# Anonymousijcai2024ttnet/scale_imagenet

Measured on AMD Instinct MI355X. Metric: images/sec ImageNet 224x224, TT-small, MI355X; top-1 exact-match, higher is better.
Workload: dtype u16/u32/u64 packed bits (gate path); f32 as prescaled fp16x2 split operands on the 16-bit MFMA (stem, lin1, lin2); 1 GPU; TT_general_imagenet_v2_small forward, batch=256 224x224 per GPU, bit-packed HIP LUT kernels (BASELINE.json configs[1]); batch_per_gpu=256, global_batch=256, batches_in_flight=2, input=float32 NCHW, normalised (the reference's contract), parallelism=batch shard x1

## Files before the change

scale_imagenet_amd/csrc/head.hip:

```cpp

#include <algorithm>
#include <cmath>
#include <type_traits>

#include "ttnet_common.h"

namespace ttnet {

namespace {

typedef float f32x16 __attribute__((ext_vector_type(16)));

typedef _Float16 f16x8 __attribute__((ext_vector_type(8)));
constexpr int NP = SPLIT_PLANES;

#ifndef TT_LIN1_SKIP
#define TT_LIN1_SKIP 0
#endif
constexpr int kLin1Skip = TT_LIN1_SKIP;

#ifndef TT_LIN1_BM
#define TT_LIN1_BM 128
#endif
#ifndef TT_LIN1_WGS
#define TT_LIN1_WGS 256
#endif
constexpr int G_BM = TT_LIN1_BM, G_BN = 128;
constexpr int G_MT = G_BM / 32, G_NT = G_BN / 32;
constexpr int G_KS = 1;
constexpr int G_CHUNK = 1024;
constexpr int G_STAGE = (G_MT + G_NT) * G_KS * NP * G_CHUNK;
#ifndef TT_LIN1_STAGES
#define TT_LIN1_STAGES 4
#endif
constexpr int G_STAGES = TT_LIN1_STAGES;
#ifndef TT_LIN1_WAVES
#define TT_LIN1_WAVES (TT_LIN1_BM / 32)
#endif
constexpr int G_WAVES = TT_LIN1_WAVES;
constexpr int G_WN = G_WAVES / G_MT, NPW = G_NT / G_WN;
static_assert(G_WAVES % G_MT == 0 && G_NT % G_WN == 0, "waves tile the workgroup's output");
constexpr int G_CHUNKS = (G_MT + G_NT) * G_KS * NP;
#ifndef TT_LIN1_LOADERS
#define TT_LIN1_LOADERS 0
#endif
constexpr int G_LOADERS = TT_LIN1_LOADERS;
constexpr int G_THREADS = 64 * (G_WAVES + G_LOADERS);
constexpr int G_LW = G_LOADERS ? G_LOADERS : G_WAVES;
constexpr int G_LOADS = (G_CHUNKS + G_LW - 1) / G_LW;
constexpr int G_LDS = G_STAGES * G_STAGE + G_CHUNK;

#ifdef TT_LIN1_STAMP
__device__ unsigned long long g_lin1_stamps[512][2];
#endif
template <int AUX_A, int AUX_B>
__global__ __launch_bounds__(G_THREADS) void gemm_f16x2_kernel(const uint8_t *__restrict__ Af, const uint8_t *__restrict__ Bf,
                                                         float *__restrict__ part, int M, int N, int KS, int ks_per,
                                                         int n_tiles, int m_tiles, int splits) {
  extern __shared__ __align__(16) uint8_t lds[];
  const int lane = threadIdx.x & 63, wave = __builtin_amdgcn_readfirstlane(threadIdx.x >> 6);
  const bool loader = G_LOADERS ? wave >= G_WAVES : true, consumer = wave < G_WAVES;
  const int lw = G_LOADERS ? (loader ? wave - G_WAVES : 0) : wave;
  int ntile, mtile, slice;
  {
    const int b = blockIdx.x, groups = m_tiles * splits;
    const int lanes8 = groups < 8 ? groups : 8;
    const int round = b / (lanes8 * n_tiles), rem = b % (lanes8 * n_tiles);
    int grp = round * lanes8 + rem % lanes8;
    ntile = rem / lanes8;
    if (round == groups / lanes8) {
      const int left = groups - round * lanes8;
      grp = round * lanes8 + rem % left;
      ntile = rem / left;
    }
    mtile = grp / splits;
    slice = grp % splits;
  }
  const int mt0 = mtile * G_MT, nt0 = ntile * G_NT;
  const int ks_beg = slice * ks_per, iters = ks_per / G_KS;

  const uint8_t *chunk_src[G_LOADS];
  int chunk_lds[G_LOADS];
#pragma unroll
  for (int jj = 0; jj < G_LOADS; ++jj) {
    const int c = lw + G_LW * jj;
    const bool real = c < G_CHUNKS;
    const bool isA = c < G_MT * G_KS * NP;
    const int cc = real ? (isA ? c : c - G_MT * G_KS * NP) : 0;
    const int pl = cc % NP, kk = (cc / NP) % G_KS, tl = cc / (NP * G_KS);
    chunk_src[jj] = (isA || !real ? Af : Bf) +
                    ((((size_t)((isA || !real ? mt0 : nt0) + tl) * KS + ks_beg + kk) * NP + pl) * 64 + lane) * 16;
    chunk_lds[jj] = real ? c * G_CHUNK : -1;
  }
  auto issue = [&](int it, int buf) {
    static_for<0, G_LOADS>([&](auto jc) {
      constexpr int jj = decltype(jc)::value;
      constexpr bool allA = G_LW * jj + G_LW - 1 < G_MT * G_KS * NP, allB = G_LW * jj >= G_MT * G_KS * NP;
      if constexpr (kLin1Skip & 3) {
        const bool isA = lw + G_LW * jj < G_MT * G_KS * NP;
        if (((kLin1Skip & 1) && isA) || ((kLin1Skip & 2) && !isA)) return;
      }
      const auto src = (const __attribute__((address_space(1))) void *)(chunk_src[jj] + (size_t)it * (G_KS * NP * G_CHUNK));
      const auto dst = (__attribute__((address_space(3))) void *)(lds + (chunk_lds[jj] >= 0 ? buf * G_STAGE + chunk_lds[jj] : G_STAGES * G_STAGE));
      if constexpr (allA) __builtin_amdgcn_global_load_lds(src, dst, 16, 0, AUX_A);
      else if constexpr (allB) __builtin_amdgcn_global_load_lds(src, dst, 16, 0, AUX_B);
      else __builtin_amdgcn_global_load_lds(src, dst, 16, 0, 0);
    });
  };

  constexpr int MPW = 1;
  const int wm = wave % G_MT, wn = wave / G_MT;
  f32x16 acc[MPW][NPW];
#pragma unroll
  for (int i = 0; i < MPW; ++i)
#pragma unroll
    for (int j = 0; j < NPW; ++j)
#pragma unroll
      for (int r = 0; r < 16; ++r) acc[i][j][r] = 0.f;

  static_assert(G_KS == 1 && MPW == 1 && NPW == 4, "the fragment pipeline below is written for one k-step per stage and four N-tiles per wave");
  auto wait_landed = [&](int younger) {
    if (younger >= 5) asm volatile("s_waitcnt vmcnt(%0)" ::"n"(5 * G_LOADS) : "memory");
    else if (younger == 4) asm volatile("s_waitcnt vmcnt(%0)" ::"n"(4 * G_LOADS) : "memory");
    else if (younger == 3) asm volatile("s_waitcnt vmcnt(%0)" ::"n"(3 * G_LOADS) : "memory");
    else if (younger == 2) asm volatile("s_waitcnt vmcnt(%0)" ::"n"(2 * G_LOADS) : "memory");
    else if (younger == 1) asm volatile("s_waitcnt vmcnt(%0)" ::"n"(G_LOADS) : "memory");
    else asm volatile("s_waitcnt vmcnt(0)" ::: "memory");
  };
  static_assert(G_STAGES >= 4 && G_STAGES <= 8 && 5 * G_LOADS < 64, "G_STAGES - 1 stages issued ahead; the barrier of k-step it frees slot (it - 1) % G_STAGES");
#ifdef TT_LIN1_STAMP
  const unsigned long long st_c = __builtin_amdgcn_s_memtime(), st_r = __builtin_amdgcn_s_memrealtime();
#endif
  if (loader) {
    for (int p = 0; p < G_STAGES - 1 && p < iters; ++p) issue(p, p);
    wait_landed(min(G_STAGES - 2, iters - 1));
  }
  __builtin_amdgcn_s_barrier();
  typedef uint32_t u32x4 __attribute__((ext_vector_type(4)));
  u32x4 af[2][NP], bq[NPW][NP];
#define TT_DSRD(dst, addr, off) asm volatile("ds_read_b128 %0, %1 offset:%2" : "=&v"(dst) : "v"(addr), "n"(off))
  const uint32_t lds0 = (uint32_t)(uintptr_t)(__attribute__((address_space(3))) void *)lds + (uint32_t)lane * 16u;
  const uint32_t offA = (uint32_t)(wm * NP) * G_CHUNK, offB = (uint32_t)(G_MT * NP + wn * NPW * NP) * G_CHUNK;
  auto tile = [&](int j, const u32x4 (&a_cur)[NP]) {
    if constexpr (kLin1Skip & 4) {
      acc[0][j][0] += __uint_as_float(a_cur[0][0] ^ bq[j][0][0] ^ bq[j][1][0] ^ a_cur[1][0]);
    } else {
      const f16x8 a0 = __builtin_bit_cast(f16x8, a_cur[0]), a1 = __builtin_bit_cast(f16x8, a_cur[1]);
      const f16x8 b0 = __builtin_bit_cast(f16x8, bq[j][0]), b1 = __builtin_bit_cast(f16x8, bq[j][1]);
      acc[0][j] = __builtin_amdgcn_mfma_f32_32x32x16_f16(a1, b0, acc[0][j], 0, 0, 0);
      acc[0][j] = __builtin_amdgcn_mfma_f32_32x32x16_f16(a0, b1, acc[0][j], 0, 0, 0);
      acc[0][j] = __builtin_amdgcn_mfma_f32_32x32x16_f16(a0, b0, acc[0][j], 0, 0, 0);
    }
    __builtin_amdgcn_sched_barrier(0);
  };
  auto kstep = [&](auto par_c, int it) {
    constexpr int P = decltype(par_c)::value;
    u32x4 (&a_cur)[NP] = af[P];
    u32x4 (&a_nxt)[NP] = af[1 - P];
    const uint32_t sb = lds0 + (uint32_t)(it % G_STAGES) * G_STAGE + offB;
    const uint32_t sn = lds0 + (uint32_t)((it + 1) % G_STAGES) * G_STAGE;
    const uint32_t snb = sn + offB, sna = sn + offA;
    TT_DSRD(bq[2][0], sb, 4 * G_CHUNK);
    TT_DSRD(bq[2][1], sb, 5 * G_CHUNK);
    asm volatile("s_waitcnt lgkmcnt(4)" : "+v"(bq[0][0]), "+v"(bq[0][1]), "+v"(a_cur[0]), "+v"(a_cur[1]));
    tile(0, a_cur);
    TT_DSRD(bq[3][0], sb, 6 * G_CHUNK);
    TT_DSRD(bq[3][1], sb, 7 * G_CHUNK);
    asm volatile("s_waitcnt lgkmcnt(4)" : "+v"(bq[1][0]), "+v"(bq[1][1]));
    tile(1, a_cur);
    TT_DSRD(bq[0][0], snb, 0);
    TT_DSRD(bq[0][1], snb, G_CHUNK);
    TT_DSRD(a_nxt[0], sna, 0);
    TT_DSRD(a_nxt[1], sna, G_CHUNK);
    asm volatile("s_waitcnt lgkmcnt(6)" : "+v"(bq[2][0]), "+v"(bq[2][1]));
    tile(2, a_cur);
    TT_DSRD(bq[1][0], snb, 2 * G_CHUNK);
    TT_DSRD(bq[1][1], snb, 3 * G_CHUNK);
    asm volatile("s_waitcnt lgkmcnt(6)" : "+v"(bq[3][0]), "+v"(bq[3][1]));
    tile(3, a_cur);
  };
  if (consumer) {
    const uint32_t s0 = lds0;
    TT_DSRD(bq[0][0], s0 + offB, 0);
    TT_DSRD(bq[0][1], s0 + offB, G_CHUNK);
    TT_DSRD(af[0][0], s0 + offA, 0);
    TT_DSRD(af[0][1], s0 + offA, G_CHUNK);
    TT_DSRD(bq[1][0], s0 + offB, 2 * G_CHUNK);
    TT_DSRD(bq[1][1], s0 + offB, 3 * G_CHUNK);
  }
  auto step = [&](auto par_c, int it) {
    if (loader) wait_landed(max(0, min(it + G_STAGES - 2, iters - 1) - (it + 1)));
    __builtin_amdgcn_s_barrier();
    if (loader && it + G_STAGES - 1 < iters) issue(it + G_STAGES - 1, (it + G_STAGES - 1) % G_STAGES);
    if (consumer) kstep(par_c, it);
  };
#pragma unroll 1
  for (int it = 0; it < iters; it += 2) {
    step(std::integral_constant<int, 0>{}, it);
    if (it + 1 < iters) step(std::integral_constant<int, 1>{}, it + 1);
  }
  if (consumer)
    asm volatile("s_waitcnt lgkmcnt(0)" : "+v"(bq[0][0]), "+v"(bq[0][1]), "+v"(bq[1][0]), "+v"(bq[1][1]), "+v"(af[0][0]), "+v"(af[0][1]),
                 "+v"(af[1][0]), "+v"(af[1][1]));
#undef TT_DSRD
#ifdef TT_LIN1_STAMP
  if (threadIdx.x == 0 && blockIdx.x < 512) {
    g_lin1_stamps[blockIdx.x][0] = __builtin_amdgcn_s_memtime() - st_c;
    g_lin1_stamps[blockIdx.x][1] = 10ull * (__builtin_amdgcn_s_memrealtime() - st_r);
  }
#endif
  if (!consumer) return;
  float4 *dst = (float4 *)part + (size_t)slice * (m_tiles * G_MT) * (n_tiles * G_NT) * 256;
#pragma unroll
  for (int i = 0; i < MPW; ++i)
#pragma unroll
    for (int j = 0; j < NPW; ++j) {
      float4 *tile = dst + ((size_t)(mt0 + wm + i) * (n_tiles * G_NT) + nt0 + wn * NPW + j) * 256 + lane;
#pragma unroll
      for (int g = 0; g < 4; ++g) {
        if ((kLin1Skip & 8) && g) continue;
        tile[g * 64] = make_float4(acc[i][j][4 * g], acc[i][j][4 * g + 1], acc[i][j][4 * g + 2], acc[i][j][4 * g + 3]);
      }
    }
}

__global__ void split_to_frag_kernel(const float *__restrict__ src, uint16_t *__restrict__ dst, int R, int K, int tiles,
                                     float prescale, int ld, int kvalid) {
  const size_t i = (size_t)blockIdx.x * blockDim.x + threadIdx.x;
  const int KS = K / 16;
  if (i >= (size_t)tiles * KS * 64 * 8) return;
  const int j = i % 8, ln = (i / 8) % 64;
  const size_t tk = i / 512;
  const int ks = tk % KS, tl = tk / KS;
  const int row = tl * 32 + (ln & 31), k = ks * 16 + 8 * (ln >> 5) + j;
  const float v = row < R && k < kvalid ? src[(size_t)row * ld + k] * prescale : 0.f;
  uint16_t h1, h2;
  split_f16x2(v, h1, h2);
  const size_t base = ((size_t)tl * KS + ks) * NP;
  dst[((base + 0) * 64 + ln) * 8 + j] = h1;
  dst[((base + 1) * 64 + ln) * 8 + j] = h2;
}

__global__ void frag_to_ref_kernel(const uint16_t *__restrict__ af, float *__restrict__ out, int n, int G, int PP) {
  const size_t t = (size_t)blockIdx.x * blockDim.x + threadIdx.x;
  const size_t per = (size_t)G * PP * 16;
  if (t >= (size_t)n * per) return;
  const int kk = t % 16, pp = (t / 16) % PP, g = (t / (16 * (size_t)PP)) % G;
  const int img = t / per;
  out[(size_t)img * per + ((size_t)(16 * g + kk)) * PP + pp] = load_feature(af, img, G * PP, g * PP + pp, kk);
}

__global__ void head_mid_kernel(const float4 *__restrict__ part, int splits, const float *__restrict__ scale,
                                const float *__restrict__ shift, uint16_t *__restrict__ mid_frag, int M, int N,
                                int polynomial, uint32_t *range_flag, int mt32, int nt32) {
  const size_t i = (size_t)blockIdx.x * blockDim.x + threadIdx.x;
  const size_t per_slice = (size_t)mt32 * nt32 * 256;
  if (i >= per_slice) return;
  const int lane = i & 63, g = (i >> 6) & 3;
  const int nt = (int)((i >> 8) % nt32), mt = (int)((i >> 8) / nt32);
  const int col = nt * 32 + (lane & 31), row0 = mt * 32 + 8 * g + 4 * (lane >> 5);
  if (col >= N || row0 >= M) return;
  double s[4] = {0.0, 0.0, 0.0, 0.0};
#pragma unroll 8
  for (int z = 0; z < splits; ++z) {
    const float4 v = part[(size_t)z * per_slice + i];
    s[0] += (double)v.x; s[1] += (double)v.y; s[2] += (double)v.z; s[3] += (double)v.w;
  }
  const float sc = scale[col], sh = shift[col];
#pragma unroll
  for (int e = 0; e < 4; ++e) {
// ... 32 lines not shown
    if (sl < nk) load(sl, fa[sl], fb[sl]);
  });
  for (int i0 = 0; i0 < nk; i0 += L2_STAGES) {
    static_for<0, L2_STAGES>([&](auto ss) {
      constexpr int sl = decltype(ss)::value;
      if (i0 + sl < nk) {
        const f16x8 a0 = __builtin_bit_cast(f16x8, fa[sl][0]), a1 = __builtin_bit_cast(f16x8, fa[sl][1]);
        const f16x8 b0 = __builtin_bit_cast(f16x8, fb[sl][0]), b1 = __builtin_bit_cast(f16x8, fb[sl][1]);
        acc = __builtin_amdgcn_mfma_f32_32x32x16_f16(a1, b0, acc, 0, 0, 0);
        acc = __builtin_amdgcn_mfma_f32_32x32x16_f16(a0, b1, acc, 0, 0, 0);
        acc = __builtin_amdgcn_mfma_f32_32x32x16_f16(a0, b0, acc, 0, 0, 0);
        if (i0 + sl + L2_STAGES < nk) load(i0 + sl + L2_STAGES, fa[sl], fb[sl]);
      }
    });
  }
#pragma unroll
  for (int r = 0; r < 16; ++r) red[(wave * 16 + r) * 64 + lane] = acc[r];
  __syncthreads();
  for (int e = threadIdx.x; e < 16 * 64; e += 64 * L2_WAVES) {
    double sum = 0.0;
#pragma unroll
    for (int w = 0; w < L2_WAVES; ++w) sum += (double)red[w * (16 * 64) + e];
    const int ln = e & 63, r = e >> 6;
    const int row = mt * 32 + (r & 3) + 8 * (r >> 2) + 4 * (ln >> 5);
    const int col = nt * 32 + (ln & 31);
    if (row < M && col < N) out[(size_t)row * N + col] = (float)(sum * (double)inv + (double)bias[col]);
  }
}

__global__ void permute_lin1_kernel(const float *__restrict__ w1, float *__restrict__ w1p, int O, int G, int PP) {
  const size_t i = (size_t)blockIdx.x * blockDim.x + threadIdx.x;
  const size_t K = (size_t)G * PP * 16;
  if (i >= (size_t)O * K) return;
  const size_t o = i / K, f = i % K;
  const int k = f % 16, pp = (f / 16) % PP, g = f / (16 * (size_t)PP);
  w1p[i] = w1[o * K + ((size_t)(16 * g + k)) * PP + pp];
}

}

int gemm_f16x2_splits(int M, int N, int KS) {
  const int tiles = ((M + G_BM - 1) / G_BM) * ((N + G_BN - 1) / G_BN);
  const int want = std::max(TT_LIN1_WGS / std::max(1, tiles), 8);
  for (int s = std::min(std::min(want, KS / 8), 128); s > 1; --s)
    if (KS % s == 0) return s;
  return 1;
}

size_t gemm_f16x2_part_elems(int M, int N, int KS) {
  const size_t mt = (M + G_BM - 1) / G_BM, nt = (N + G_BN - 1) / G_BN;
  return (size_t)gemm_f16x2_splits(M, N, KS) * mt * G_BM * nt * G_BN;
}

int launch_gemm_f16x2(const void *Af, const void *Bf, float *part, int M, int N, int K, int splits, hipStream_t s) {
  const int KS = K / 16;
  if (K % 16 || KS % splits || (KS / splits) % G_KS) {
    set_error("gemm_f16x2: K=%d not divisible into %d slices of %d k-steps", K, splits, G_KS);
    return TTNET_E_UNSUPPORTED;
  }
  static const int nt = getenv("TTNET_LIN1_NT") ? atoi(getenv("TTNET_LIN1_NT")) : 0;
  const int n_tiles = (N + G_BN - 1) / G_BN, m_tiles = (M + G_BM - 1) / G_BM;
  auto launch = [&](auto kernel) -> int {
    TT_TRY(ensure_dynamic_lds((const void *)kernel, G_LDS));
    hipLaunchKernelGGL(kernel, dim3(n_tiles * m_tiles * splits), dim3(G_THREADS), G_LDS, s, (const uint8_t *)Af, (const uint8_t *)Bf, part, M, N,
                       KS, KS / splits, n_tiles, m_tiles, splits);
    return TTNET_OK;
  };
  if (nt == 11) TT_TRY(launch(gemm_f16x2_kernel<2, 2>));
  else if (nt == 1) TT_TRY(launch(gemm_f16x2_kernel<0, 2>));
  else if (nt == 10) TT_TRY(launch(gemm_f16x2_kernel<2, 0>));
  else TT_TRY(launch(gemm_f16x2_kernel<0, 0>));
  TT_HIP(hipGetLastError());
  return TTNET_OK;
}

size_t frag_elems(int rows, int K) { return (size_t)((rows + 31) / 32) * (K / 16) * NP * 64 * 8; }

float weight_prescale(const float *w, size_t n) {
  float amax = 0.f;
  for (size_t i = 0; i < n; ++i) amax = fmaxf(amax, fabsf(w[i]));
  if (!(amax > 0.f) || !std::isfinite(amax)) return 1.0f;
  int e;
  frexpf(amax, &e);
  int k = 14 - e;
  k = k > 60 ? 60 : (k < -60 ? -60 : k);
  return ldexpf(1.0f, k);
}

int launch_split_to_frag(const float *src, void *dst, int R, int K, int rows_padded, float prescale, hipStream_t s, int ld,
                         int kvalid) {
  if (K % 16) {
    set_error("split_to_frag: K=%d is not a multiple of 16", K);
    return TTNET_E_UNSUPPORTED;
  }
  const int tiles = (rows_padded + 31) / 32;
  const size_t t = (size_t)tiles * (K / 16) * 64 * 8;
  hipLaunchKernelGGL(split_to_frag_kernel, dim3((unsigned)((t + 255) / 256)), dim3(256), 0, s, src, (uint16_t *)dst, R, K, tiles,
                     prescale, ld > 0 ? ld : K, kvalid > 0 ? kvalid : K);
  TT_HIP(hipGetLastError());
  return TTNET_OK;
}

int launch_frag_to_reference_order(const void *af, float *out, int n, int G, int PP, hipStream_t s) {
  const size_t t = (size_t)n * G * PP * 16;
  hipLaunchKernelGGL(frag_to_ref_kernel, dim3((unsigned)((t + 255) / 256)), dim3(256), 0, s, (const uint16_t *)af, out, n, G, PP);
  TT_HIP(hipGetLastError());
  return TTNET_OK;
}

int launch_head_mid(const float *part, int splits, const float *scale, const float *shift, void *mid_frag, int M, int N,
                    int polynomial, uint32_t *range_flag, hipStream_t s) {
  const int mt32 = (M + G_BM - 1) / G_BM * G_MT, nt32 = (N + G_BN - 1) / G_BN * G_NT;
  const size_t t = (size_t)mt32 * nt32 * 256;
  hipLaunchKernelGGL(head_mid_kernel, dim3((unsigned)((t + 255) / 256)), dim3(256), 0, s, (const float4 *)part, splits, scale, shift,
                     (uint16_t *)mid_frag, M, N, polynomial, range_flag, mt32, nt32);
  TT_HIP(hipGetLastError());
  return TTNET_OK;
}

int launch_lin2_f16x2(const void *mid_frag, const void *w2f, const float *bias, float inv, float *out, int M, int N, int K,
                      hipStream_t s) {
  const int KS = (K + 15) / 16;
  hipLaunchKernelGGL(lin2_f16x2_kernel, dim3((N + 31) / 32, (M + 31) / 32), dim3(64 * L2_WAVES), 0, s,
                     (const uint4 *)mid_frag, (const uint4 *)w2f, bias, inv, out, M, N, KS);
// ... 19 lines not shown
```

scale_imagenet_amd/csrc/plan.hip:

```cpp

#include <math.h>
#include <stdarg.h>
#include <stdint.h>
#include <stdio.h>
#include <stdlib.h>
#include <string.h>

#include <algorithm>
#include <array>
#include <map>
#include <mutex>
#include <unordered_map>

#include "ttnet_common.h"

namespace ttnet {

static thread_local char g_err[1024] = "";

void set_error(const char *fmt, ...) {
  va_list ap;
  va_start(ap, fmt);
  vsnprintf(g_err, sizeof(g_err), fmt, ap);
  va_end(ap);
// ... 80 lines not shown
  float *full_gel = nullptr;

  uint16_t *stem_wt = nullptr;
  float *stem_init = nullptr;
  uint32_t *norm_tab = nullptr;
  uint16_t *stem_wt_u8 = nullptr;
  float *stem_init_u8 = nullptr;
  float in_mean[3] = {0.485f, 0.456f, 0.406f}, in_std[3] = {0.229f, 0.224f, 0.225f};
  float *w1p = nullptr;
  uint16_t *w1f = nullptr;
  float *bn_scale = nullptr, *bn_shift = nullptr;
  uint16_t *w2f = nullptr;
  float lin2_inv = 1.f;
  size_t part_elems = 0;
  size_t table_bytes = 0, workspace_bytes = 0;
  bool usage_on = false;
  size_t usage_bytes = 0;
  int usage_scheme_dw = kUsageMerged, usage_scheme_pw = kUsageMerged;

  bool profiling = false;
  struct GraphEntry {
    hipGraph_t graph = nullptr;
    hipGraphExec_t exec = nullptr;
    struct Kernel {
      hipGraphNode_t node = nullptr;
      hipKernelNodeParams p{};
      uint64_t argv[12] = {};
      void *args[12] = {};
    };
    Kernel first, last;
    const void *x = nullptr;
    void *out = nullptr;
  };
  struct Lane {
    struct Block {
      uint16_t *o[4] = {nullptr, nullptr, nullptr, nullptr};
      uint64_t *c3_tmp = nullptr;
      uint32_t *idx = nullptr;
    };
    std::vector<uint64_t *> x_rp;
    std::vector<uint16_t *> x_cp;
    std::vector<Block> blk;
    uint64_t *va_y = nullptr;
    float *last_float = nullptr;
    uint32_t *full_fix = nullptr;
    float *part = nullptr;
    uint16_t *feat = nullptr;
    uint16_t *mid_frag = nullptr;
    uint64_t *u_rows = nullptr, *u_br[4] = {nullptr, nullptr, nullptr, nullptr};
    uint32_t *u_tap = nullptr;
    std::map<int64_t, GraphEntry> graphs;
    std::map<int64_t, int> eager_calls;
    int64_t last_n = 0;
  };
  std::vector<Lane> lanes;
  int last_lane = 0;
  hipStream_t cap_stream = nullptr;
  bool graphs_ok = getenv("TTNET_NO_GRAPH") == nullptr;
  int64_t graph_replays = 0;
  int64_t graph_captures = 0, graph_drops = 0;
  std::string graph_off_reason;
  uint32_t *range_host = nullptr, *range_dev = nullptr;
  std::vector<Timing> timings;
  size_t timing_used = 0;

  std::vector<void *> owned;
};

int ttnet::ensure_dynamic_lds(const void *kernel, size_t bytes) {
  if (bytes <= 64 * 1024) return TTNET_OK;
  static std::mutex mu;
  static std::unordered_map<const void *, size_t> done;
  std::lock_guard<std::mutex> lock(mu);
  auto it = done.find(kernel);
  if (it != done.end() && it->second >= bytes) return TTNET_OK;
  TT_HIP(hipFuncSetAttribute(kernel, hipFuncAttributeMaxDynamicSharedMemorySize, (int)bytes));
  done[kernel] = bytes;
  return TTNET_OK;
}

namespace {

template <typename T>
int dev_alloc(ttnet_plan *pl, T **out, size_t count, bool zero, size_t *account = nullptr) {
  void *ptr = nullptr;
  const size_t bytes = std::max<size_t>(count * sizeof(T), 16);
  hipError_t e = hipMalloc(&ptr, bytes);
  if (e != hipSuccess) {
    set_error("hipMalloc(%zu bytes) failed: %s", bytes, hipGetErrorString(e));
    return TTNET_E_NOMEM;
  }
  if (zero) TT_HIP(hipMemset(ptr, 0, bytes));
  pl->owned.push_back(ptr);
  if (account) *account += bytes;
  *out = (T *)ptr;
  return TTNET_OK;
}

void dev_free(ttnet_plan *pl, void *ptr) {
  if (!ptr) return;
  auto it = std::find(pl->owned.begin(), pl->owned.end(), ptr);
  if (it != pl->owned.end()) pl->owned.erase(it);
  (void)hipFree(ptr);
}

void add_tensor(ttnet_plan *pl, const std::string &key, std::vector<int64_t> shape, int dtype, bool required) {
// ... 582 lines not shown
  }
  {
    FullPwArgs a = pw_args(mh.c3, mh.H, mh.W);
    a.interleaved = 0; a.src[0] = L.x_rp[i];
    a.out_rp = c3_tmp; a.out_float = nullptr;
    static const char *const kC3[4] = {"full.conv3.f4", "full.conv3.f5", "full.conv3.f6", "full.conv3.f7"};
    TT_TIMED(pl, kC3[std::min<size_t>(i, 3)], s, launch_full_pw(a, s));
    TT_TIMED(pl, "full.maj3", s,
             launch_rp_majority(c3_tmp, o64[2], n, mh.C, mh.H, mh.W, mh.Ho, mh.off34, mh.off34, s));
    TT_TIMED(pl, "full.maj4", s,
             launch_rp_majority(L.x_rp[i], o64[3], n, mh.C, mh.H, mh.W, mh.Ho, mh.off34, mh.off34, s));
  }
  {
    FullPwArgs a = pw_args(mh.cf, mh.Ho, mh.Wo);
    a.interleaved = 1;
    for (int k = 0; k < 4; ++k) a.src[k] = o64[k];
    if (mh.last) {
      a.out_rp = nullptr; a.out_float = L.last_float;
      TT_TIMED(pl, "full.convf_last", s, launch_full_pw(a, s));
      TT_TIMED(pl, "full.pool", s, launch_full_pool_split(L.last_float, L.feat, n, mh.cf.g.out_planes, mh.Ho, mh.Wo, pl->range_dev, s));
    } else {
      a.out_rp = L.x_rp[i + 1]; a.out_float = nullptr;
      static const char *const kCf[4] = {"full.convf.f4", "full.convf.f5", "full.convf.f6", "full.convf.f7"};
      TT_TIMED(pl, kCf[std::min<size_t>(i, 3)], s, launch_full_pw(a, s));
    }
  }
  return TTNET_OK;
}

int prepare_head(ttnet_plan *pl, hipStream_t s) {
  const Tensor &t1 = pl->tensors[pl->head + ".lin1.weight"], &t2 = pl->tensors[pl->head + ".lin2.weight"];
  std::vector<double> sc, sh;
  TT_TRY(fold_bn(pl, pl->head + ".BN2", sc, sh));
  std::vector<float> w;
  TT_TRY(fetch(t1, w));
  const float ws1 = weight_prescale(w.data(), w.size());
  for (double &v : sc) v /= (double)ws1 * ACT_PRESCALE;
  TT_TRY(upload_f32(pl->bn_scale, sc));
  TT_TRY(upload_f32(pl->bn_shift, sh));
  const float *w1 = (const float *)t1.dev;
  if (pl->path != GatePath::VAlexnet) {
    TT_TRY(launch_permute_lin1(w1, pl->w1p, pl->inter, pl->featC / 16, pl->featPP, s));
    w1 = pl->w1p;
  }
  TT_TRY(launch_split_to_frag(w1, pl->w1f, pl->inter, pl->fcsize, (pl->inter + 127) / 128 * 128, ws1, s));
  TT_TRY(fetch(t2, w));
  const float ws2 = weight_prescale(w.data(), w.size());
  pl->lin2_inv = 1.0f / (ws2 * ACT_PRESCALE);
  const int kpad = (pl->inter + 15) / 16 * 16;
  return launch_split_to_frag((const float *)t2.dev, pl->w2f, pl->n_classes, kpad, (pl->n_classes + 63) / 64 * 64, ws2, s, pl->inter,
                              pl->inter);
}

int run_head(ttnet_plan *pl, const ttnet_plan::Lane &L, int n, float *logits, hipStream_t s) {
  const int polynomial = pl->path == GatePath::VAlexnet ? 0 : 1;
  const int s1 = gemm_f16x2_splits(n, pl->inter, pl->fcsize / 16);
  TT_TIMED(pl, "head.lin1", s, launch_gemm_f16x2(L.feat, pl->w1f, L.part, n, pl->inter, pl->fcsize, s1, s));
  TT_TIMED(pl, polynomial ? "head.bn_poly" : "head.bn", s,
           launch_head_mid(L.part, s1, pl->bn_scale, pl->bn_shift, L.mid_frag, n, pl->inter, polynomial, pl->range_dev, s));
  TT_TIMED(pl, "head.lin2", s,
           launch_lin2_f16x2(L.mid_frag, pl->w2f, (const float *)pl->tensors[pl->head + ".lin2.bias"].dev, pl->lin2_inv, logits, n,
                             pl->n_classes, pl->inter, s));
  return TTNET_OK;
}

int run_from_blocks(ttnet_plan *pl, ttnet_plan::Lane &L, int n, float *logits, hipStream_t s) {
  for (size_t i = 0; i < pl->blocks.size(); ++i) {
    switch (pl->path) {
      case GatePath::TwoLaunch: TT_TRY(run_two_launch_block(pl, L, i, n, s)); break;
      case GatePath::Fused: TT_TRY(run_fused_block(pl, L, i, n, s)); break;
      case GatePath::XSmall: TT_TRY(run_xs_block(pl, L, i, n, s)); break;
      case GatePath::Full: TT_TRY(run_full_block(pl, L, i, n, s)); break;
      case GatePath::VAlexnet: TT_TRY(run_va_block(pl, L, n, s)); break;
    }
  }
  TT_TRY(run_head(pl, L, n, logits, s));
  L.last_n = n;
  return TTNET_OK;
}

int check_range(ttnet_plan *pl) {
  if (pl->range_host && *(volatile uint32_t *)pl->range_host) {
    set_error("an earlier forward on this plan met an activation outside the range of the fp16 x 2 operand split "
              "(|input| or |feature| >= 4094, or NaN): its logits are invalid; ttnet_plan_query(\"range_overflow\") "
              "reads and clears the flag");
    return TTNET_E_RANGE;
  }
  return TTNET_OK;
}

int check_ready(ttnet_plan *pl, const void *in, int64_t n, const void *out) {
  if (!pl || !in || !out) {
    set_error("null argument");
    return TTNET_E_INVALID;
  }
  if (!pl->finalized) {
    set_error("ttnet_forward before ttnet_plan_finalize");
    return TTNET_E_STATE;
  }
  if (n < 1 || n > pl->desc.max_batch) {
    set_error("batch %lld outside [1, max_batch=%d]", (long long)n, pl->desc.max_batch);
    return TTNET_E_INVALID;
  }
  return check_range(pl);
}

BlockTT *find_block(ttnet_plan *pl, const char *name) {
  for (BlockTT *b : all_block_tts(pl))
    if (b->g.name == name) return b;
  return nullptr;
// ... 203 lines not shown
  if (lane < 0 || lane >= (int)pl->lanes.size()) {
    set_error("forward: lane %d but the plan has %d (ttnet_plan_set_lanes)", lane, (int)pl->lanes.size());
    return TTNET_E_INVALID;
  }
  pl->last_lane = lane;
  ttnet_plan::Lane &L = pl->lanes[lane];
  hipStream_t s = (hipStream_t)stream;
  if (pl->profiling || !pl->graphs_ok) return forward_eager(pl, L, x_dev, u8, n, logits_dev, s);
  const int64_t key = 2 * n + (u8 ? 1 : 0);
  hipStreamCaptureStatus cs = hipStreamCaptureStatusNone;
  if (s && hipStreamIsCapturing(s, &cs) == hipSuccess && cs != hipStreamCaptureStatusNone)
    return forward_eager(pl, L, x_dev, u8, n, logits_dev, s);
  auto it = L.graphs.find(key);
  if (it == L.graphs.end()) {
    if (++L.eager_calls[key] <= 2) return forward_eager(pl, L, x_dev, u8, n, logits_dev, s);
    ttnet_plan::GraphEntry e;
    int cap_status = TTNET_OK;
    if (!capture_forward(pl, L, x_dev, u8, n, logits_dev, e, &cap_status)) {
      drop_graph(e);
      if (cap_status != TTNET_OK) {
        --L.eager_calls[key];
        return cap_status;
      }
      graphs_off(pl, "capture or instantiation of the forward failed");
      return forward_eager(pl, L, x_dev, u8, n, logits_dev, s);
    }
    pl->graph_captures++;
    if (L.graphs.size() >= 8) {
      TT_HIP(hipDeviceSynchronize());
      drop_graph(L.graphs.begin()->second);
      L.graphs.erase(L.graphs.begin());
      pl->graph_drops++;
    }
    it = L.graphs.emplace(key, e).first;
  }
  ttnet_plan::GraphEntry &e = it->second;
  bool ok = true;
  if (e.x != x_dev) {
    ok = patch_pointer(e.exec, e.first, 0, x_dev);
    e.x = x_dev;
  }
  if (ok && e.out != logits_dev) {
    ok = patch_pointer(e.exec, e.last, kLastKernelOutArg, logits_dev);
    e.out = logits_dev;
  }
  if (ok) ok = hipGraphLaunch(e.exec, s) == hipSuccess;
  if (!ok) {
    drop_graph(e);
    L.graphs.erase(it);
    graphs_off(pl, "hipGraphExecKernelNodeSetParams / hipGraphLaunch failed");
    return forward_eager(pl, L, x_dev, u8, n, logits_dev, s);
  }
  L.last_n = n;
  pl->timing_used = 0;
  pl->graph_replays++;
  return TTNET_OK;
}

}

extern "C" {

const char *ttnet_last_error(void) { return g_err; }
const char *ttnet_version(void) { return "ttnet-mi355x 0.1 (gfx950)"; }

int ttnet_plan_create(const ttnet_net_desc *desc, int device, ttnet_plan **out) {
  if (!desc || !out) {
    set_error("null argument");
    return TTNET_E_INVALID;
  }
  *out = nullptr;
  int count = 0;
  if (hipGetDeviceCount(&count) != hipSuccess || count < 1) {
    set_error("no HIP device: libttnet has no CPU path");
    return TTNET_E_HIP;
  }
  if (device < 0 || device >= count) {
    set_error("device %d out of range (%d devices)", device, count);
    return TTNET_E_INVALID;
  }
  TT_HIP(hipSetDevice(device));
  ttnet_plan *pl = new ttnet_plan();
  pl->desc = *desc;
  pl->device = device;
  int st = build_geometry(pl);
  if (st == TTNET_OK) st = allocate(pl);
  if (st != TTNET_OK) {
    ttnet_plan_destroy(pl);
    return st;
  }
  *out = pl;
  return TTNET_OK;
}

int ttnet_plan_set_tensor(ttnet_plan *pl, const char *key, const void *ptr, const int64_t *shape, int ndim,
                          int dtype, int on_device) {
  if (!pl || !key || !ptr || (ndim > 0 && !shape)) {
    set_error("null argument");
    return TTNET_E_INVALID;
  }
  std::string k(key);
  if (k.rfind("module.", 0) == 0) k = k.substr(7);
  auto it = pl->tensors.find(k);
  if (it == pl->tensors.end()) {
    set_error("unexpected key in state_dict: %s", key);
    return TTNET_E_INVALID;
// ... 316 lines not shown
int ttnet_plan_set_table(ttnet_plan *pl, const char *name, const void *src_host, size_t src_bytes) {
  BlockTT *b = nullptr;
  TT_TRY(table_block(pl, name, src_host, src_bytes, false, &b));
  std::vector<uint8_t> raw(b->g.table_bytes(), 0);
  walk_table(*b, raw.data(), const_cast<void *>(src_host), true);
  TT_HIP(hipSetDevice(pl->device));
  TT_TRY(invalidate_graphs(pl));
  TT_HIP(hipMemcpy(b->table, raw.data(), raw.size(), hipMemcpyHostToDevice));
  b->user_table = true;
  b->near_ties = -1;
  if (pl->path == GatePath::Fused)
    for (auto &mh : pl->blocks)
      if (b == &mh.c1 || b == &mh.c2 || b == &mh.c3) {
        TT_TRY(launch_fused_images(mh.c1.table, mh.c2.table, mh.c3.table, mh.C, mh.img_dw, mh.img_c3, nullptr));
        TT_HIP(hipDeviceSynchronize());
      }
  return TTNET_OK;
}

int ttnet_plan_query(ttnet_plan *pl, const char *what, int64_t *out) {
  if (!pl || !what || !out) {
    set_error("null argument");
    return TTNET_E_INVALID;
  }
  const std::string w(what);
  if (w == "fcsize") *out = pl->fcsize;
  else if (w == "n_classes") *out = pl->n_classes;
  else if (w == "n_state_tensors") *out = (int64_t)pl->key_order.size();
  else if (w == "max_batch") *out = pl->desc.max_batch;
  else if (w == "table_bytes") *out = (int64_t)pl->table_bytes;
  else if (w == "workspace_bytes") *out = (int64_t)pl->workspace_bytes;
  else if (w == "usage_bytes") *out = (int64_t)pl->usage_bytes;
  else if (w == "p") *out = pl->p;
  else if (w == "graph_replays") *out = pl->graph_replays;
  else if (w == "graphs_enabled") {
    *out = pl->graphs_ok ? 1 : 0;
    if (!pl->graphs_ok)
      set_error("graphs disabled: %s", pl->graph_off_reason.empty() ? "TTNET_NO_GRAPH is set" : pl->graph_off_reason.c_str());
  }
  else if (w == "graph_captures") *out = pl->graph_captures;
  else if (w == "graph_drops") *out = pl->graph_drops;
  else if (w == "graphs_cached") {
    int64_t c = 0;
    for (auto &l : pl->lanes) c += (int64_t)l.graphs.size();
    *out = c;
  }
  else if (w == "range_overflow") {
    TT_HIP(hipSetDevice(pl->device));
    TT_HIP(hipDeviceSynchronize());
    *out = *(volatile uint32_t *)pl->range_host ? 1 : 0;
    *pl->range_host = 0u;
  }
  else if (w == "lanes") *out = (int64_t)pl->lanes.size();
  else if (w == "gate_path") *out = (int64_t)pl->path;
  else if (w.rfind("gate_grid:", 0) == 0) {
    char *end = nullptr;
    const long i = strtol(w.c_str() + 10, &end, 10);
    const int n = (int)pl->lanes[pl->last_lane].last_n;
    if (end == w.c_str() + 10 || *end || i < 0 || (size_t)i >= pl->blocks.size() || n <= 0 ||
        (pl->path != GatePath::Fused && pl->path != GatePath::TwoLaunch)) {
      set_error("%s: needs a block index below %zu, a forward on the lane used last, and the two-launch or fused path", what,
                pl->blocks.size());
      return TTNET_E_INVALID;
    }
    const int C = pl->blocks[(size_t)i].C;
    *out = pl->path == GatePath::Fused ? (int64_t)(C / 8) * fused_block_slices(C, n) : (int64_t)gate_stage1_grid(C, n);
  }
  else if (w == "full_listed_pw" || w == "full_listed_dw") {
    uint32_t v[2] = {0, 0};
    const uint32_t *fix = pl->lanes[pl->last_lane].full_fix;
    if (fix) {
      TT_HIP(hipSetDevice(pl->device));
      TT_HIP(hipDeviceSynchronize());
      TT_HIP(hipMemcpy(v, fix + 62, sizeof(v), hipMemcpyDeviceToHost));
    }
    *out = v[w == "full_listed_dw" ? 1 : 0];
  }
  else if (w.rfind("near_ties:", 0) == 0) {
    BlockTT *b = find_block(pl, w.c_str() + 10);
    if (!b) {
      set_error("no Block_TT named %s", w.c_str() + 10);
      return TTNET_E_INVALID;
    }
    *out = b->near_ties;
  } else {
    set_error("unknown query %s", what);
    return TTNET_E_INVALID;
  }
  return TTNET_OK;
}

int ttnet_plan_set_profiling(ttnet_plan *pl, int enabled) {
  if (!pl) {
    set_error("null plan");
    return TTNET_E_INVALID;
  }
  pl->profiling = enabled != 0;
  pl->timing_used = 0;
  return TTNET_OK;
}

int ttnet_plan_last_timings(ttnet_plan *pl, const char **names, float *ms, int cap) {
  if (!pl || !names || !ms) {
    set_error("null argument");
    return TTNET_E_INVALID;
  }
// ... 31 lines not shown
```

scale_imagenet_amd/csrc/ttnet_common.h:

```cpp
#pragma once

#include <hip/hip_runtime.h>
#include <stdint.h>
#include <string.h>
#include <algorithm>
#include <string>
#include <type_traits>
#include <vector>

#include "../../include/ttnet.h"

namespace ttnet {

void set_error(const char *fmt, ...);

#define TT_HIP(call)                                                                       \
  do {                                                                                     \
    hipError_t e__ = (call);                                                               \
    if (e__ != hipSuccess) {                                                               \
      ::ttnet::set_error("%s failed: %s (%s:%d)", #call, hipGetErrorString(e__), __FILE__, \
                         __LINE__);                                                        \
      return TTNET_E_HIP;                                                                  \
    }                                                                                      \
  } while (0)
// ... 227 lines not shown
int launch_narrow_rows(const uint64_t *src, void *dst, size_t count, int W, hipStream_t s);
int launch_xs_branches(const GateBlockArgs &a, const void *t_c3, uint64_t *const o[4], hipStream_t s);
int launch_xs_pf(int n, int C, int Ho, int Wo, int cout_g, uint64_t *const o[4], const void *t_cf, uint64_t *out_rp,
                 hipStream_t s);
int launch_xs_last(int n, int C, int Ho, int Wo, int cout_g, uint64_t *const o[4], const float *t_last, void *feat_frag,
                   uint32_t *range_flag, hipStream_t s);
struct FullDwArgs {
  int n, C, H, W;
  int kh, kw, stride, pad;
  int ho, wo;
  int Ho;
  int pad_t, pad_l;
  const uint64_t *x_rp;
  const float *w1, *w2;
  const double *s1, *t1, *s2, *t2;
  uint64_t *out;
  uint32_t *fix_list, *fix_count;
  uint32_t fix_cap;
  float tau_scale;
  const float *gel;
};
struct FullPwArgs {
  int n, H, W;
  int groups, cin, mid, cout, Cout;
  int Csrc;
  int interleaved;
  const uint64_t *src[4];
  const float *w1, *w2;
  const double *s1, *t1, *s2, *t2;
  uint64_t *out_rp;
  float *out_float;
  uint32_t *fix_list, *fix_count, *range_flag;
  float tau_scale;
  const float *gel;
};
int launch_full_dw(const FullDwArgs &a, hipStream_t s);
int launch_full_pw(const FullPwArgs &a, hipStream_t s);
size_t full_gelu_tables_elems();
int launch_full_gelu_tables(float *dst, hipStream_t s);
int launch_rp_majority(const uint64_t *x, uint64_t *out, int n, int C, int H, int W, int Ho, int pad_t, int pad_l,
                       hipStream_t s);
int launch_full_pool_split(const float *x, void *feat_frag, int n, int C, int H, int W, uint32_t *range_flag, hipStream_t s);
int launch_va_stem(const float *x, const float *w, const float *bias, const float *scale, const float *shift,
                   uint64_t *rp, int n, hipStream_t s);
int va_stem_kernel_arg_sizes(const int **sizes);
int launch_va_block(const uint64_t *x_rp, const void *t1, const void *t2, const void *t3, uint64_t *y, int n, hipStream_t s);
int launch_va_feat(const uint64_t *y, void *feat_frag, int n, hipStream_t s);
int launch_va_frag_to_flat(const void *af, float *out, int n, hipStream_t s);
int launch_cp_to_rp(const uint16_t *cp, uint64_t *rp, int n, int C, int H, int W, hipStream_t s);
int launch_rp_to_cp(const uint64_t *rp, uint16_t *cp, int n, int C, int H, int W, hipStream_t s);
int launch_frag_to_reference_order(const void *af, float *out, int n, int G, int PP, hipStream_t s);
int gemm_f16x2_splits(int M, int N, int KS);
size_t gemm_f16x2_part_elems(int M, int N, int KS);
int launch_gemm_f16x2(const void *Af, const void *Bf, float *part, int M, int N, int K, int splits, hipStream_t s);
size_t frag_elems(int rows, int K);
int launch_split_to_frag(const float *src, void *dst, int R, int K, int rows_padded, float prescale, hipStream_t s, int ld = 0,
                         int kvalid = 0);

int launch_head_mid(const float *part, int splits, const float *scale, const float *shift, void *mid_frag, int M, int N,
                    int polynomial, uint32_t *range_flag, hipStream_t s);
int launch_lin2_f16x2(const void *mid_frag, const void *w2f, const float *bias, float inv, float *out, int M, int N, int K,
                      hipStream_t s);
int lin2_kernel_arg_sizes(const int **sizes);
int launch_permute_lin1(const float *w1, float *w1p, int O, int G, int PP, hipStream_t s);

constexpr int kUsagePlain = 0, kUsageMerged = 1;
int launch_usage_dw(const uint64_t *x_rp, int n, int C, int H, int W, int Ho, int Wo, int kh, int kw, int stride, int pad,
                    int64_t *counters, int scheme, hipStream_t s);
int launch_usage_pw(const uint64_t *const *src, int nsrc, int n, int Csrc, int groups, int cin_g, int H, int W, int64_t *counters,
                    int scheme, hipStream_t s);

}
```

Before: 1.973 million images/s.

## Add 256-row lin1 GEMM tile with two M-tiles per wave for multi-lane plans

Adds a 256-row workgroup tile variant to the fp16x2 lin1 GEMM. Each of four waves now owns two 32-row M-tiles across all four N-tiles, and the LDS read schedule is hand-interleaved so B fragments are reused across both M-tiles. The plan selects this tile when at least two lanes are in flight, the gate path is neither Full nor VAlexnet, and the 128-row tile count is even. The aim is to halve B-fragment LDS traffic and global loads per output and cut workgroup count, in exchange for more accumulator registers, a larger LDS footprint and fewer workgroups to fill the GPU.

Result: slower. 1.922 million images/s (-2.6%).

```diff
diff --git a/scale_imagenet_amd/csrc/head.hip b/scale_imagenet_amd/csrc/head.hip
--- a/scale_imagenet_amd/csrc/head.hip
+++ b/scale_imagenet_amd/csrc/head.hip
@@ -25,38 +25,40 @@
 #ifndef TT_LIN1_WGS
 #define TT_LIN1_WGS 256
 #endif
-constexpr int G_BM = TT_LIN1_BM, G_BN = 128;
+constexpr int G_BM = 128, G_BN = 128;
 constexpr int G_MT = G_BM / 32, G_NT = G_BN / 32;
 constexpr int G_KS = 1;
 constexpr int G_CHUNK = 1024;
-constexpr int G_STAGE = (G_MT + G_NT) * G_KS * NP * G_CHUNK;
 #ifndef TT_LIN1_STAGES
 #define TT_LIN1_STAGES 4
 #endif
 constexpr int G_STAGES = TT_LIN1_STAGES;
-#ifndef TT_LIN1_WAVES
-#define TT_LIN1_WAVES (TT_LIN1_BM / 32)
-#endif
-constexpr int G_WAVES = TT_LIN1_WAVES;
-constexpr int G_WN = G_WAVES / G_MT, NPW = G_NT / G_WN;
-static_assert(G_WAVES % G_MT == 0 && G_NT % G_WN == 0, "waves tile the workgroup's output");
-constexpr int G_CHUNKS = (G_MT + G_NT) * G_KS * NP;
+constexpr int G_WAVES = 4, NPW = G_NT;
 #ifndef TT_LIN1_LOADERS
 #define TT_LIN1_LOADERS 0
 #endif
 constexpr int G_LOADERS = TT_LIN1_LOADERS;
 constexpr int G_THREADS = 64 * (G_WAVES + G_LOADERS);
 constexpr int G_LW = G_LOADERS ? G_LOADERS : G_WAVES;
-constexpr int G_LOADS = (G_CHUNKS + G_LW - 1) / G_LW;
-constexpr int G_LDS = G_STAGES * G_STAGE + G_CHUNK;
+template <int BM>
+struct Lin1Tile {
+  static_assert(BM == 128 || BM == 256, "one or two M-tiles of 32 rows per wave");
+  static constexpr int MT = BM / 32, MPW = MT / G_WAVES;
+  static constexpr int CHUNKS = (MT + G_NT) * G_KS * NP;
+  static constexpr int STAGE = CHUNKS * G_CHUNK;
+  static constexpr int LOADS = (CHUNKS + G_LW - 1) / G_LW;
+  static constexpr int LDS = G_STAGES * STAGE + G_CHUNK;
+};
 
 #ifdef TT_LIN1_STAMP
 __device__ unsigned long long g_lin1_stamps[512][2];
 #endif
-template <int AUX_A, int AUX_B>
+template <int AUX_A, int AUX_B, int BM = TT_LIN1_BM>
 __global__ __launch_bounds__(G_THREADS) void gemm_f16x2_kernel(const uint8_t *__restrict__ Af, const uint8_t *__restrict__ Bf,
                                                          float *__restrict__ part, int M, int N, int KS, int ks_per,
                                                          int n_tiles, int m_tiles, int splits) {
+  using T = Lin1Tile<BM>;
+  constexpr int G_MT = T::MT, MPW = T::MPW, G_CHUNKS = T::CHUNKS, G_STAGE = T::STAGE, G_LOADS = T::LOADS;
   extern __shared__ __align__(16) uint8_t lds[];
   const int lane = threadIdx.x & 63, wave = __builtin_amdgcn_readfirstlane(threadIdx.x >> 6);
   const bool loader = G_LOADERS ? wave >= G_WAVES : true, consumer = wave < G_WAVES;
@@ -108,8 +110,7 @@
     });
   };
 
-  constexpr int MPW = 1;
-  const int wm = wave % G_MT, wn = wave / G_MT;
+  const int wm = wave % G_WAVES;
   f32x16 acc[MPW][NPW];
 #pragma unroll
   for (int i = 0; i < MPW; ++i)
@@ -118,7 +119,7 @@
 #pragma unroll
       for (int r = 0; r < 16; ++r) acc[i][j][r] = 0.f;
 
-  static_assert(G_KS == 1 && MPW == 1 && NPW == 4, "the fragment pipeline below is written for one k-step per stage and four N-tiles per wave");
+  static_assert(G_KS == 1 && (MPW == 1 || MPW == 2) && NPW == 4, "the fragment pipeline below is written for one k-step per stage, one or two M-tiles and four N-tiles per wave");
   auto wait_landed = [&](int younger) {
     if (younger >= 5) asm volatile("s_waitcnt vmcnt(%0)" ::"n"(5 * G_LOADS) : "memory");
     else if (younger == 4) asm volatile("s_waitcnt vmcnt(%0)" ::"n"(4 * G_LOADS) : "memory");
@@ -137,56 +138,99 @@
   }
   __builtin_amdgcn_s_barrier();
   typedef uint32_t u32x4 __attribute__((ext_vector_type(4)));
-  u32x4 af[2][NP], bq[NPW][NP];
+  u32x4 af[2][MPW][NP], bq[NPW][NP];
 #define TT_DSRD(dst, addr, off) asm volatile("ds_read_b128 %0, %1 offset:%2" : "=&v"(dst) : "v"(addr), "n"(off))
   const uint32_t lds0 = (uint32_t)(uintptr_t)(__attribute__((address_space(3))) void *)lds + (uint32_t)lane * 16u;
-  const uint32_t offA = (uint32_t)(wm * NP) * G_CHUNK, offB = (uint32_t)(G_MT * NP + wn * NPW * NP) * G_CHUNK;
-  auto tile = [&](int j, const u32x4 (&a_cur)[NP]) {
+  const uint32_t offA = (uint32_t)(wm * NP) * G_CHUNK, offB = (uint32_t)(G_MT * NP) * G_CHUNK;
+  constexpr uint32_t offA1 = (uint32_t)(G_WAVES * NP) * G_CHUNK;
+  auto tile = [&](auto i_c, int j, const u32x4 (&a_cur)[NP]) {
+    constexpr int i = decltype(i_c)::value;
     if constexpr (kLin1Skip & 4) {
-      acc[0][j][0] += __uint_as_float(a_cur[0][0] ^ bq[j][0][0] ^ bq[j][1][0] ^ a_cur[1][0]);
+      acc[i][j][0] += __uint_as_float(a_cur[0][0] ^ bq[j][0][0] ^ bq[j][1][0] ^ a_cur[1][0]);
     } else {
       const f16x8 a0 = __builtin_bit_cast(f16x8, a_cur[0]), a1 = __builtin_bit_cast(f16x8, a_cur[1]);
       const f16x8 b0 = __builtin_bit_cast(f16x8, bq[j][0]), b1 = __builtin_bit_cast(f16x8, bq[j][1]);
-      acc[0][j] = __builtin_amdgcn_mfma_f32_32x32x16_f16(a1, b0, acc[0][j], 0, 0, 0);
-      acc[0][j] = __builtin_amdgcn_mfma_f32_32x32x16_f16(a0, b1, acc[0][j], 0, 0, 0);
-      acc[0][j] = __builtin_amdgcn_mfma_f32_32x32x16_f16(a0, b0, acc[0][j], 0, 0, 0);
+      acc[i][j] = __builtin_amdgcn_mfma_f32_32x32x16_f16(a1, b0, acc[i][j], 0, 0, 0);
+      acc[i][j] = __builtin_amdgcn_mfma_f32_32x32x16_f16(a0, b1, acc[i][j], 0, 0, 0);
+      acc[i][j] = __builtin_amdgcn_mfma_f32_32x32x16_f16(a0, b0, acc[i][j], 0, 0, 0);
     }
     __builtin_amdgcn_sched_barrier(0);
   };
+  constexpr std::integral_constant<int, 0> m0{};
+  constexpr std::integral_constant<int, MPW - 1> m1{};
   auto kstep = [&](auto par_c, int it) {
     constexpr int P = decltype(par_c)::value;
-    u32x4 (&a_cur)[NP] = af[P];
-    u32x4 (&a_nxt)[NP] = af[1 - P];
+    u32x4 (&a_cur)[MPW][NP] = af[P];
+    u32x4 (&a_nxt)[MPW][NP] = af[1 - P];
     const uint32_t sb = lds0 + (uint32_t)(it % G_STAGES) * G_STAGE + offB;
     const uint32_t sn = lds0 + (uint32_t)((it + 1) % G_STAGES) * G_STAGE;
     const uint32_t snb = sn + offB, sna = sn + offA;
-    TT_DSRD(bq[2][0], sb, 4 * G_CHUNK);
-    TT_DSRD(bq[2][1], sb, 5 * G_CHUNK);
-    asm volatile("s_waitcnt lgkmcnt(4)" : "+v"(bq[0][0]), "+v"(bq[0][1]), "+v"(a_cur[0]), "+v"(a_cur[1]));
-    tile(0, a_cur);
-    TT_DSRD(bq[3][0], sb, 6 * G_CHUNK);
-    TT_DSRD(bq[3][1], sb, 7 * G_CHUNK);
-    asm volatile("s_waitcnt lgkmcnt(4)" : "+v"(bq[1][0]), "+v"(bq[1][1]));
-    tile(1, a_cur);
-    TT_DSRD(bq[0][0], snb, 0);
-    TT_DSRD(bq[0][1], snb, G_CHUNK);
-    TT_DSRD(a_nxt[0], sna, 0);
-    TT_DSRD(a_nxt[1], sna, G_CHUNK);
-    asm volatile("s_waitcnt lgkmcnt(6)" : "+v"(bq[2][0]), "+v"(bq[2][1]));
-    tile(2, a_cur);
-    TT_DSRD(bq[1][0], snb, 2 * G_CHUNK);
-    TT_DSRD(bq[1][1], snb, 3 * G_CHUNK);
-    asm volatile("s_waitcnt lgkmcnt(6)" : "+v"(bq[3][0]), "+v"(bq[3][1]));
-    tile(3, a_cur);
+    if constexpr (MPW == 1) {
+      TT_DSRD(bq[2][0], sb, 4 * G_CHUNK);
+      TT_DSRD(bq[2][1], sb, 5 * G_CHUNK);
+      asm volatile("s_waitcnt lgkmcnt(4)" : "+v"(bq[0][0]), "+v"(bq[0][1]), "+v"(a_cur[0][0]), "+v"(a_cur[0][1]));
+      tile(m0, 0, a_cur[0]);
+      TT_DSRD(bq[3][0], sb, 6 * G_CHUNK);
+      TT_DSRD(bq[3][1], sb, 7 * G_CHUNK);
+      asm volatile("s_waitcnt lgkmcnt(4)" : "+v"(bq[1][0]), "+v"(bq[1][1]));
+      tile(m0, 1, a_cur[0]);
+      TT_DSRD(bq[0][0], snb, 0);
+      TT_DSRD(bq[0][1], snb, G_CHUNK);
+      TT_DSRD(a_nxt[0][0], sna, 0);
+      TT_DSRD(a_nxt[0][1], sna, G_CHUNK);
+      asm volatile("s_waitcnt lgkmcnt(6)" : "+v"(bq[2][0]), "+v"(bq[2][1]));
+      tile(m0, 2, a_cur[0]);
+      TT_DSRD(bq[1][0], snb, 2 * G_CHUNK);
+      TT_DSRD(bq[1][1], snb, 3 * G_CHUNK);
+      asm volatile("s_waitcnt lgkmcnt(6)" : "+v"(bq[3][0]), "+v"(bq[3][1]));
+      tile(m0, 3, a_cur[0]);
+    } else {
+      TT_DSRD(bq[2][0], sb, 4 * G_CHUNK);
+      TT_DSRD(bq[2][1], sb, 5 * G_CHUNK);
+      asm volatile("s_waitcnt lgkmcnt(6)" : "+v"(bq[0][0]), "+v"(bq[0][1]), "+v"(a_cur[0][0]), "+v"(a_cur[0][1]));
+      tile(m0, 0, a_cur[0]);
+      TT_DSRD(bq[3][0], sb, 6 * G_CHUNK);
+      TT_DSRD(bq[3][1], sb, 7 * G_CHUNK);
+      asm volatile("s_waitcnt lgkmcnt(6)" : "+v"(a_cur[MPW - 1][0]), "+v"(a_cur[MPW - 1][1]));
+      tile(m1, 0, a_cur[MPW - 1]);
+      TT_DSRD(a_nxt[0][0], sna, 0);
+      TT_DSRD(a_nxt[0][1], sna, G_CHUNK);
+      asm volatile("s_waitcnt lgkmcnt(6)" : "+v"(bq[1][0]), "+v"(bq[1][1]));
+      tile(m0, 1, a_cur[0]);
+      TT_DSRD(bq[0][0], snb, 0);
+      TT_DSRD(bq[0][1], snb, G_CHUNK);
+      tile(m1, 1, a_cur[MPW - 1]);
+      TT_DSRD(a_nxt[MPW - 1][0], sna, offA1);
+      TT_DSRD(a_nxt[MPW - 1][1], sna, offA1 + G_CHUNK);
+      asm volatile("s_waitcnt lgkmcnt(8)" : "+v"(bq[2][0]), "+v"(bq[2][1]));
+      tile(m0, 2, a_cur[0]);
+      TT_DSRD(bq[1][0], snb, 2 * G_CHUNK);
+      TT_DSRD(bq[1][1], snb, 3 * G_CHUNK);
+      tile(m1, 2, a_cur[MPW - 1]);
+      asm volatile("s_waitcnt lgkmcnt(8)" : "+v"(bq[3][0]), "+v"(bq[3][1]));
+      tile(m0, 3, a_cur[0]);
+      tile(m1, 3, a_cur[MPW - 1]);
+    }
   };
   if (consumer) {
     const uint32_t s0 = lds0;
-    TT_DSRD(bq[0][0], s0 + offB, 0);
-    TT_DSRD(bq[0][1], s0 + offB, G_CHUNK);
-    TT_DSRD(af[0][0], s0 + offA, 0);
-    TT_DSRD(af[0][1], s0 + offA, G_CHUNK);
-    TT_DSRD(bq[1][0], s0 + offB, 2 * G_CHUNK);
-    TT_DSRD(bq[1][1], s0 + offB, 3 * G_CHUNK);
+    if constexpr (MPW == 1) {
+      TT_DSRD(bq[0][0], s0 + offB, 0);
+      TT_DSRD(bq[0][1], s0 + offB, G_CHUNK);
+      TT_DSRD(af[0][0][0], s0 + offA, 0);
+      TT_DSRD(af[0][0][1], s0 + offA, G_CHUNK);
+      TT_DSRD(bq[1][0], s0 + offB, 2 * G_CHUNK);
+      TT_DSRD(bq[1][1], s0 + offB, 3 * G_CHUNK);
+    } else {
+      TT_DSRD(af[0][0][0], s0 + offA, 0);
+      TT_DSRD(af[0][0][1], s0 + offA, G_CHUNK);
+      TT_DSRD(bq[0][0], s0 + offB, 0);
+      TT_DSRD(bq[0][1], s0 + offB, G_CHUNK);
+      TT_DSRD(af[0][MPW - 1][0], s0 + offA, offA1);
+      TT_DSRD(af[0][MPW - 1][1], s0 + offA, offA1 + G_CHUNK);
+      TT_DSRD(bq[1][0], s0 + offB, 2 * G_CHUNK);
+      TT_DSRD(bq[1][1], s0 + offB, 3 * G_CHUNK);
+    }
   }
   auto step = [&](auto par_c, int it) {
     if (loader) wait_landed(max(0, min(it + G_STAGES - 2, iters - 1) - (it + 1)));
@@ -200,8 +244,10 @@
     if (it + 1 < iters) step(std::integral_constant<int, 1>{}, it + 1);
   }
   if (consumer)
-    asm volatile("s_waitcnt lgkmcnt(0)" : "+v"(bq[0][0]), "+v"(bq[0][1]), "+v"(bq[1][0]), "+v"(bq[1][1]), "+v"(af[0][0]), "+v"(af[0][1]),
-                 "+v"(af[1][0]), "+v"(af[1][1]));
+    asm volatile("s_waitcnt lgkmcnt(0)" : "+v"(bq[0][0]), "+v"(bq[0][1]), "+v"(bq[1][0]), "+v"(bq[1][1]), "+v"(af[0][0][0]), "+v"(af[0][0][1]),
+                 "+v"(af[1][0][0]), "+v"(af[1][0][1]));
+  if constexpr (MPW == 2)
+    if (consumer) asm volatile("" : "+v"(af[0][1][0]), "+v"(af[0][1][1]), "+v"(af[1][1][0]), "+v"(af[1][1][1]));
 #undef TT_DSRD
 #ifdef TT_LIN1_STAMP
   if (threadIdx.x == 0 && blockIdx.x < 512) {
@@ -215,7 +261,7 @@
   for (int i = 0; i < MPW; ++i)
 #pragma unroll
     for (int j = 0; j < NPW; ++j) {
-      float4 *tile = dst + ((size_t)(mt0 + wm + i) * (n_tiles * G_NT) + nt0 + wn * NPW + j) * 256 + lane;
+      float4 *tile = dst + ((size_t)(mt0 + wm + G_WAVES * i) * (n_tiles * G_NT) + nt0 + j) * 256 + lane;
 #pragma unroll
       for (int g = 0; g < 4; ++g) {
         if ((kLin1Skip & 8) && g) continue;
@@ -354,24 +400,31 @@
   return (size_t)gemm_f16x2_splits(M, N, KS) * mt * G_BM * nt * G_BN;
 }
 
-int launch_gemm_f16x2(const void *Af, const void *Bf, float *part, int M, int N, int K, int splits, hipStream_t s) {
+int launch_gemm_f16x2(const void *Af, const void *Bf, float *part, int M, int N, int K, int splits, hipStream_t s, int tile_rows) {
   const int KS = K / 16;
   if (K % 16 || KS % splits || (KS / splits) % G_KS) {
     set_error("gemm_f16x2: K=%d not divisible into %d slices of %d k-steps", K, splits, G_KS);
     return TTNET_E_UNSUPPORTED;
   }
+  if (tile_rows == 0) tile_rows = TT_LIN1_BM;
+  const int m128 = (M + G_BM - 1) / G_BM;
+  if ((tile_rows != 128 && tile_rows != 256) || (tile_rows == 256 && m128 % 2)) {
+    set_error("gemm_f16x2: a tile of %d rows does not fit M=%d (128, or 256 with an even number of 128-row tiles)", tile_rows, M);
+    return TTNET_E_UNSUPPORTED;
+  }
   static const int nt = getenv("TTNET_LIN1_NT") ? atoi(getenv("TTNET_LIN1_NT")) : 0;
-  const int n_tiles = (N + G_BN - 1) / G_BN, m_tiles = (M + G_BM - 1) / G_BM;
-  auto launch = [&](auto kernel) -> int {
-    TT_TRY(ensure_dynamic_lds((const void *)kernel, G_LDS));
-    hipLaunchKernelGGL(kernel, dim3(n_tiles * m_tiles * splits), dim3(G_THREADS), G_LDS, s, (const uint8_t *)Af, (const uint8_t *)Bf, part, M, N,
-                       KS, KS / splits, n_tiles, m_tiles, splits);
+  const int n_tiles = (N + G_BN - 1) / G_BN, m_tiles = m128 * G_BM / tile_rows;
+  auto launch = [&](auto kernel, int lds_bytes) -> int {
+    TT_TRY(ensure_dynamic_lds((const void *)kernel, lds_bytes));
+    hipLaunchKernelGGL(kernel, dim3(n_tiles * m_tiles * splits), dim3(G_THREADS), lds_bytes, s, (const uint8_t *)Af, (const uint8_t *)Bf, part, M,
+                       N, KS, KS / splits, n_tiles, m_tiles, splits);
     return TTNET_OK;
   };
-  if (nt == 11) TT_TRY(launch(gemm_f16x2_kernel<2, 2>));
-  else if (nt == 1) TT_TRY(launch(gemm_f16x2_kernel<0, 2>));
-  else if (nt == 10) TT_TRY(launch(gemm_f16x2_kernel<2, 0>));
-  else TT_TRY(launch(gemm_f16x2_kernel<0, 0>));
+  if (tile_rows == 256) TT_TRY(launch(gemm_f16x2_kernel<0, 0, 256>, Lin1Tile<256>::LDS));
+  else if (nt == 11) TT_TRY(launch(gemm_f16x2_kernel<2, 2, 128>, Lin1Tile<128>::LDS));
+  else if (nt == 1) TT_TRY(launch(gemm_f16x2_kernel<0, 2, 128>, Lin1Tile<128>::LDS));
+  else if (nt == 10) TT_TRY(launch(gemm_f16x2_kernel<2, 0, 128>, Lin1Tile<128>::LDS));
+  else TT_TRY(launch(gemm_f16x2_kernel<0, 0, 128>, Lin1Tile<128>::LDS));
   TT_HIP(hipGetLastError());
   return TTNET_OK;
 }
diff --git a/scale_imagenet_amd/csrc/plan.hip b/scale_imagenet_amd/csrc/plan.hip
--- a/scale_imagenet_amd/csrc/plan.hip
+++ b/scale_imagenet_amd/csrc/plan.hip
@@ -156,6 +156,7 @@
     std::map<int64_t, GraphEntry> graphs;
     std::map<int64_t, int> eager_calls;
     int64_t last_n = 0;
+    int last_lin1_rows = 0;
   };
   std::vector<Lane> lanes;
   int last_lane = 0;
@@ -844,10 +845,19 @@
                               pl->inter);
 }
 
-int run_head(ttnet_plan *pl, const ttnet_plan::Lane &L, int n, float *logits, hipStream_t s) {
+int lin1_tile_rows(const ttnet_plan *pl, int n) {
+  static const int wide_env = getenv("TTNET_LIN1_WIDE") ? atoi(getenv("TTNET_LIN1_WIDE")) : -1;
+  const bool pairs = ((n + 127) / 128) % 2 == 0;
+  const bool wide = wide_env >= 0 ? wide_env != 0
+                                  : pl->lanes.size() >= 2 && pl->path != GatePath::Full && pl->path != GatePath::VAlexnet;
+  return wide && pairs ? 256 : 128;
+}
+
+int run_head(ttnet_plan *pl, ttnet_plan::Lane &L, int n, float *logits, hipStream_t s) {
   const int polynomial = pl->path == GatePath::VAlexnet ? 0 : 1;
   const int s1 = gemm_f16x2_splits(n, pl->inter, pl->fcsize / 16);
-  TT_TIMED(pl, "head.lin1", s, launch_gemm_f16x2(L.feat, pl->w1f, L.part, n, pl->inter, pl->fcsize, s1, s));
+  L.last_lin1_rows = lin1_tile_rows(pl, n);
+  TT_TIMED(pl, "head.lin1", s, launch_gemm_f16x2(L.feat, pl->w1f, L.part, n, pl->inter, pl->fcsize, s1, s, L.last_lin1_rows));
   TT_TIMED(pl, polynomial ? "head.bn_poly" : "head.bn", s,
            launch_head_mid(L.part, s1, pl->bn_scale, pl->bn_shift, L.mid_frag, n, pl->inter, polynomial, pl->range_dev, s));
   TT_TIMED(pl, "head.lin2", s,
@@ -1157,6 +1167,7 @@
     return forward_eager(pl, L, x_dev, u8, n, logits_dev, s);
   }
   L.last_n = n;
+  L.last_lin1_rows = lin1_tile_rows(pl, (int)n);
   pl->timing_used = 0;
   pl->graph_replays++;
   return TTNET_OK;
@@ -1579,6 +1590,7 @@
     *pl->range_host = 0u;
   }
   else if (w == "lanes") *out = (int64_t)pl->lanes.size();
+  else if (w == "lin1_tile_rows") *out = pl->lanes[pl->last_lane].last_lin1_rows;
   else if (w == "gate_path") *out = (int64_t)pl->path;
   else if (w.rfind("gate_grid:", 0) == 0) {
     char *end = nullptr;
diff --git a/scale_imagenet_amd/csrc/ttnet_common.h b/scale_imagenet_amd/csrc/ttnet_common.h
--- a/scale_imagenet_amd/csrc/ttnet_common.h
+++ b/scale_imagenet_amd/csrc/ttnet_common.h
@@ -303,7 +303,8 @@
 int launch_frag_to_reference_order(const void *af, float *out, int n, int G, int PP, hipStream_t s);
 int gemm_f16x2_splits(int M, int N, int KS);
 size_t gemm_f16x2_part_elems(int M, int N, int KS);
-int launch_gemm_f16x2(const void *Af, const void *Bf, float *part, int M, int N, int K, int splits, hipStream_t s);
+int launch_gemm_f16x2(const void *Af, const void *Bf, float *part, int M, int N, int K, int splits, hipStream_t s,
+                      int tile_rows = 0);
 size_t frag_elems(int rows, int K);
 int launch_split_to_frag(const float *src, void *dst, int R, int K, int rows_padded, float prescale, hipStream_t s, int ld = 0,
                          int kvalid = 0);
```
